# klebgenomics/Kaptive

Measured on AMD Instinct MI355X. Metric: assemblies typed/sec (K+O), higher is better.
Workload: dtype uint16x2 (exact; int32-equivalent); 1 GPU; 10000 synthetic 5 Mbp kpsc assemblies per GPU typed against the synthetic K-locus database, then the O-locus database; one step = all of them, as 10 batches of 1000 through context-owned work buffers; packed assemblies resident in HBM before the timed region; one alignment pass over the genes of both databases, one reduction per database; alignment_passes_per_batch=1, assemblies_per_gpu=10000, assemblies_total=10000, batch=1000, parallelism=1 x independent shard, no collective

## Files before the change

### kaptive_amd/csrc/kp_align.hip

```cpp
#include "kp_host.h"

static const char *const NO_RESULTS = "this batch has no resident alignment results (not aligned yet, or displaced: a context keeps the results of its KP_WORK_SLOTS most recently aligned batches)";

static int enqueue_forked(kp_ctx *ctx, kp_batch *b, KpWork *w, hipStream_t stream) {
    const KpAnchors an = w->anchors();
    const KpTasks tasks = w->tasks();
    const KpJoins joins = w->joins();
    const KpTrace trace = w->trace();
    kp_launch_join_chain(an, tasks, w->groups(), joins, w->d_jscratch.p, ctx->opt.join, w->jstream);
    kp_launch_join_fill(b->view, ctx->genes, joins, trace, ctx->opt.join, w->jstream);
    kp_launch_join_trace(b->view, ctx->genes, joins, tasks, trace, ctx->opt.join, w->jstream);
    kp_launch_task_order(b->view, ctx->genes, an, tasks, stream);
    KP_HIP_CHECK(ctx, hipEventRecord(w->ev[KP_EV_ORDER], stream));
    kp_launch_sw(b->view, ctx->genes, tasks, trace, ctx->max_gene_len > KP_FILL16_MAX_GENE_LEN, ctx->opt.trace_summary, stream, w->ev[KP_EV_FILL]);
    KP_HIP_CHECK(ctx, hipEventRecord(w->ev[KP_EV_TRACEBACK], stream));
    return KP_OK;
}

static int enqueue_align(kp_ctx *ctx, kp_batch *b, KpWork *w) {
    const size_t n_asm = w->n_asm;
    for (auto &e : w->ev)
        if (!e) KP_HIP_CHECK(ctx, hipEventCreate(&e.h));
    if (!w->astream) KP_HIP_CHECK(ctx, hipStreamCreateWithFlags(&w->astream.h, hipStreamNonBlocking));
    if (!w->jstream) {
        KP_HIP_CHECK(ctx, hipStreamCreateWithFlags(&w->jstream.h, hipStreamNonBlocking));
        KP_HIP_CHECK(ctx, hipEventCreateWithFlags(&w->ev_jfork.h, hipEventDisableTiming));
        KP_HIP_CHECK(ctx, hipEventCreateWithFlags(&w->ev_jdone.h, hipEventDisableTiming));
    }
    hipStream_t stream = w->astream;
    const Event *ev = w->ev;
    if ((uint64_t)n_asm * w->anchor_cap > 0xFFFFFFF0ull)
        return kp_fail(ctx, KP_EOVERFLOW, "anchor buffer would exceed 2^32 entries; use smaller batches");
    if (((uint64_t)b->view.total_words << 4) >> KP_CAND_POS_BITS)
        return kp_fail(ctx, KP_EOVERFLOW, "a batch holds at most 2^33 bases (candidate positions); use smaller batches");
    KP_HIP_CHECK(ctx, w->d_anchors_a.reserve(n_asm * w->anchor_cap));
    KP_HIP_CHECK(ctx, w->d_anchors_b.reserve(n_asm * w->anchor_cap));
    KP_HIP_CHECK(ctx, w->d_counts.reserve(w->counts_len()));
// ... 500 lines not shown
```

### kaptive_amd/csrc/kp_ctx.hip

```cpp
#include <cctype>
#include <cstdlib>
#include <mutex>
#include <new>
#include <unordered_map>
#include <sys/mman.h>

#include "kp_host.h"

static std::mutex g_err_mutex;
static std::string g_global_error = "";

std::atomic<long long> g_dev_allocs{0};
bool g_debug_alloc = false;

static std::mutex g_pin_mutex;
struct PinBlock { size_t bytes; bool mapped, locked; };
static std::unordered_map<void *, PinBlock> g_pin_blocks;
static size_t g_pin_bytes = 0;
constexpr size_t HUGE_PAGE = (size_t)2 << 20;
hipError_t pinned_alloc(void **out, size_t bytes) {
    const hipError_t e = hipHostMalloc(out, bytes, hipHostMallocPortable);
    if (e == hipSuccess) {
        std::lock_guard<std::mutex> lk(g_pin_mutex);
        g_pin_blocks[*out] = PinBlock{bytes, false, true};
// ... 72 lines not shown
    const long long x = std::atoll(v);
    return x > 0 ? (uint32_t)x : dflt;
}

static void options_from_env(KpOptions &o) {
    o.anchor_cap = env_u32("KAPTIVE_AMD_ANCHOR_CAP", o.anchor_cap);
    o.tasks_per_asm = env_u32("KAPTIVE_AMD_TASKS_PER_ASM", o.tasks_per_asm);
    o.hit_cap = env_u32("KAPTIVE_AMD_HIT_CAP", o.hit_cap);
    o.trace_kb_per_asm = env_u32("KAPTIVE_AMD_TRACE_KB_PER_ASM", o.trace_kb_per_asm);
    o.trace_set = env_u32("KAPTIVE_AMD_TRACE_KB_PER_ASM", 0) != 0;
    o.cand_cap = env_u32("KAPTIVE_AMD_CAND_CAP", 0);
    o.group_cap = env_u32("KAPTIVE_AMD_GROUP_CAP", o.group_cap);
    o.join_cap = env_u32("KAPTIVE_AMD_JOIN_CAP", o.join_cap);
    o.occ_slots = env_u32("KAPTIVE_AMD_OCC_SLOTS", o.occ_slots);
    o.kept_cap = env_u32("KAPTIVE_AMD_KEPT_CAP", o.kept_cap);
    o.piece_cap = env_u32("KAPTIVE_AMD_PIECE_CAP", o.piece_cap);
    o.prot_cap = env_u32("KAPTIVE_AMD_PROT_CAP", o.prot_cap);
    o.scan_mode = (int)env_u32("KAPTIVE_AMD_SCAN_ABLATE", 0);
    o.library_sort = (int)env_u32("KAPTIVE_AMD_LIBRARY_SORT", 0);
    o.upload_piece_mb = std::max<uint32_t>(1, env_u32("KAPTIVE_AMD_UPLOAD_PIECE_MB", 4096));
    { const char *rb = getenv("KAPTIVE_AMD_READBACK"); o.readback_copy_engine = rb && std::string(rb) == "copy"; }
    o.spin_wait = (int)env_u32("KAPTIVE_AMD_SPIN_WAIT", 0);
    { const char *ts = std::getenv("KAPTIVE_AMD_TRACE_SUMMARY"); o.trace_summary = !(ts && std::string(ts) == "0"); }
    o.join_stats = std::getenv("KAPTIVE_AMD_JOIN_STATS") != nullptr;
    if (const char *e = std::getenv("KAPTIVE_AMD_JOIN_GRID")) std::sscanf(e, "%d,%d,%d,%d", &o.join.fill, &o.join.walk, &o.join.chain, &o.join.chain_large);
    if (const char *e = std::getenv("KAPTIVE_AMD_JOIN_PRIO")) o.join.prio = std::atoi(e);
    if (const char *e = std::getenv("KAPTIVE_AMD_SKIP_JOINS")) o.join.skip = std::atoi(e);
    g_debug_alloc = std::getenv("KAPTIVE_AMD_DEBUG_ALLOC") != nullptr;
}

static void fill_blosum(int8_t *m) {
    static const int8_t b[25][25] = {
        {4, -1, -2, -2, 0, -1, -1, 0, -2, -1, -1, -1, -1, -2, -1, 1, 0, -3, -2, 0, -2, -1, -1, -1, -4},
        {-1, 5, 0, -2, -3, 1, 0, -2, 0, -3, -2, 2, -1, -3, -2, -1, -1, -3, -2, -3, -1, -2, 0, -1, -4},
        {-2, 0, 6, 1, -3, 0, 0, 0, 1, -3, -3, 0, -2, -3, -2, 1, 0, -4, -2, -3, 4, -3, 0, -1, -4},
        {-2, -2, 1, 6, -3, 0, 2, -1, -1, -3, -4, -1, -3, -3, -1, 0, -1, -4, -3, -3, 4, -3, 1, -1, -4},
        {0, -3, -3, -3, 9, -3, -4, -3, -3, -1, -1, -3, -1, -2, -3, -1, -1, -2, -2, -1, -3, -1, -3, -1, -4},
        {-1, 1, 0, 0, -3, 5, 2, -2, 0, -3, -2, 1, 0, -3, -1, 0, -1, -2, -1, -2, 0, -2, 4, -1, -4},
        {-1, 0, 0, 2, -4, 2, 5, -2, 0, -3, -3, 1, -2, -3, -1, 0, -1, -3, -2, -2, 1, -3, 4, -1, -4},
        {0, -2, 0, -1, -3, -2, -2, 6, -2, -4, -4, -2, -3, -3, -2, 0, -2, -2, -3, -3, -1, -4, -2, -1, -4},
        {-2, 0, 1, -1, -3, 0, 0, -2, 8, -3, -3, -1, -2, -1, -2, -1, -2, -2, 2, -3, 0, -3, 0, -1, -4},
        {-1, -3, -3, -3, -1, -3, -3, -4, -3, 4, 2, -3, 1, 0, -3, -2, -1, -3, -1, 3, -3, 3, -3, -1, -4},
        {-1, -2, -3, -4, -1, -2, -3, -4, -3, 2, 4, -2, 2, 0, -3, -2, -1, -2, -1, 1, -4, 3, -3, -1, -4},
        {-1, 2, 0, -1, -3, 1, 1, -2, -1, -3, -2, 5, -1, -3, -1, 0, -1, -3, -2, -2, 0, -3, 1, -1, -4},
        {-1, -1, -2, -3, -1, 0, -2, -3, -2, 1, 2, -1, 5, 0, -2, -1, -1, -1, -1, 1, -3, 2, -1, -1, -4},
        {-2, -3, -3, -3, -2, -3, -3, -3, -1, 0, 0, -3, 0, 6, -4, -2, -2, 1, 3, -1, -3, 0, -3, -1, -4},
// ... 84 lines not shown
    if (ctx) return ctx->error.c_str();
    std::lock_guard<std::mutex> lk(g_err_mutex);
    static thread_local std::string copy;
    copy = g_global_error;
    return copy.c_str();
}

void *kp_ctx_stream(kp_ctx *ctx) { return ctx ? (void *)ctx->stream.h : nullptr; }

int kp_ctx_set_option(kp_ctx *ctx, const char *name, int64_t value) {
    if (!ctx) return kp_fail(nullptr, KP_EINVAL, "null context");
    if (!name || value < 0) return kp_fail(ctx, KP_EINVAL, "bad option");
    const std::string n(name);
    KpOptions &o = ctx->opt;
    if (kp_caps_set_option(o, ctx->learnt, ctx->run_caps, n, value)) return KP_OK;
    if (kp_caps_set_cs_option(ctx->cs_caps, n, value)) return KP_OK;
    if (kp_caps_set_variants_option(ctx->var_caps, n, value)) return KP_OK;
    if (n == "scan_mode") o.scan_mode = (int)value;
    else if (n == "library_sort") o.library_sort = value != 0;
    else if (n == "cigar") o.cigar = value != 0;
    else if (n == "cs") o.cs = value != 0;
    else if (n == "variants") o.variants = value != 0;
    else if (n == "aligned") o.aligned = value != 0;
    else if (n == "upload_piece_mb") o.upload_piece_mb = (uint32_t)std::max<int64_t>(1, std::min<int64_t>(value, 4096));
    else return kp_fail(ctx, KP_EINVAL, "unknown option: " + n);
    return KP_OK;
}

int kp_host_alloc(size_t bytes, void **out) {
    if (!out) return kp_fail(nullptr, KP_EINVAL, "out is null");
    *out = nullptr;
    if (bytes >= 4 * HUGE_PAGE) {
        int rc = kp_host_reserve(bytes, out);
        if (rc == KP_OK && (rc = kp_host_lock(*out)) == KP_OK) return KP_OK;
        if (*out) { pinned_free(*out); *out = nullptr; }
    }
    const hipError_t e = pinned_alloc(out, std::max<size_t>(bytes, 1));
    if (e != hipSuccess) return kp_fail(nullptr, KP_ENOMEM, std::string("hipHostMalloc: ") + hipGetErrorString(e));
    return KP_OK;
}

int kp_host_reserve(size_t bytes, void **out) {
    if (!out) return kp_fail(nullptr, KP_EINVAL, "out is null");
    *out = mapped_alloc(std::max<size_t>(bytes, 1));
    if (!*out) return kp_fail(nullptr, KP_ENOMEM, "mmap failed");
    return KP_OK;
// ... 20 lines not shown
```

### kaptive_amd/csrc/kp_host.h

```cpp
#pragma once

#include <cstring>
#include <memory>
#include "kp_internal.h"
#include "kp_caps.h"
#include "kp_device.h"
#include "kp_reduce_core.h"
static_assert(KP_CAPS_ANCHOR_SUBS == KP_ANCHOR_SUBS, "the policy sizes the scan's sub-slices");

struct KpTypingGroup {
    int32_t gene_lo = 0, gene_hi = 0;
    DevBuf<uint16_t> d_gene_locus, d_gene_pos;
    DevBuf<uint8_t> d_gene_extra, d_prot_db;
    DevBuf<int8_t> d_gene_strand;
    DevBuf<int32_t> d_locus_off, d_locus_len, d_prot_db_off, d_prot_db_len;
    KpTypingDb typing{};
    int max_db_prot_len = 0;
};

struct KpRowLayout {
    bool valid = false;
    size_t n_asm = 0;
    std::vector<int64_t> h_off;
    DevBuf<int64_t> d_off;
// ... 79 lines not shown
    size_t slots() const { return n_asm * (size_t)kept_cap; }
    size_t pairs_len() const { return 4 * slots() + n_asm + 1; }
    KpReduceTables tables() const {
        int32_t *const q = d_pairs.p, *const base = q + 4 * slots();
        return {.best = d_best.p, .keys = d_keys.p, .order = d_order.p, .kept_flag = d_flag.p, .kept = d_kept.p, .kept_cap = kept_cap,
                .pieces = d_pieces.p, .piece_cap = piece_cap, .summary = d_summary.p, .prot = d_prot.p, .prot_cap = prot_cap,
                .q_off = q, .q_len = q + slots(), .t_off = q + 2 * slots(), .t_len = q + 3 * slots(), .pair_base = base, .n_pairs = base + n_asm, .dp8 = d_dp.p};
    }
};

struct kp_batch;

struct KpOptions : KpCapOptions {
    int scan_mode = 0;
    int library_sort = 0;
    uint32_t upload_piece_mb = 4096;
    int readback_copy_engine = 0;
    int spin_wait = 0;
    int cigar = 0;
    int variants = 0;
    int aligned = 0;
    int cs = 0;
    bool trace_summary = true;
    bool join_stats = false;
    KpJoinLaunch join;
};

struct KpInput {
    DevBuf<uint32_t> d_words;
    DevBuf<int64_t> d_asm_word_off;
    DevBuf<int32_t> d_ctg_start, d_ctg_len, d_asm_first_ctg, d_n_runs, d_asm_first_nrun;
    PinnedBlock h_stage;
    Event ready;
};

enum KpPassEvent { KP_EV_START, KP_EV_SCAN, KP_EV_SORT, KP_EV_ORDER, KP_EV_FILL, KP_EV_TRACEBACK, KP_EV_JOINED, KP_EV_END, KP_N_EVENTS };
static_assert(KP_EV_END == 7, "kp_batch_profile returns seven stage times");
enum KpStat { KP_STAT_ANCHORS, KP_STAT_TASKS, KP_STAT_CELLS, KP_STAT_HITS, KP_STAT_RERUNS, KP_N_STATS };
enum KpTopWord { KP_TOP_TRACE = 0, KP_TOP_OCC = 3, KP_TOP_WORDS = 4 };
enum KpJoinCount { KP_JOIN_GROUPS = 0, KP_JOIN_CLASSES = 1, KP_JOIN_COUNTS = 1 + KP_N_CLASSES };
enum KpCandCount { KP_CAND_FRONT, KP_CAND_BACK, KP_CAND_COUNTS };

struct KpWork : KpPassCaps {
    kp_batch *owner = nullptr;
    size_t n_asm = 0;
    KpKeyBits key_bits{16, 30};
// ... 201 lines not shown
```

### kaptive_amd/csrc/kp_internal.h

```cpp
#pragma once

#include <hip/hip_runtime.h>
#include <stdint.h>

#include <string>
#include <vector>

#include "../../include/kaptive_amd.h"

#define KP_FILTER_LOG2 24
__host__ __device__ inline uint32_t kp_filter_block(uint32_t x) { return x & ((1u << (KP_FILTER_LOG2 - 6)) - 1u); }
__host__ __device__ inline uint2 kp_filter_mask2(uint32_t x) {
    uint2 m;
    m.x = 1u << ((x >> 18) & 31u);
    m.y = 1u << ((x >> 23) & 31u);
    return m;
}
__host__ __device__ inline bool kp_filter_test(uint2 got, uint32_t x) {
    return ((got.x >> ((x >> 18) & 31u)) & (got.y >> ((x >> 23) & 31u)) & 1u) != 0u;
}
__host__ __device__ inline uint64_t kp_filter_mask(uint32_t kmer) {
    const uint2 m = kp_filter_mask2(kmer);
    return ((uint64_t)m.y << 32) | m.x;
}
// ... 180 lines not shown
struct KpPieceRows { const kp_piece *pieces; int piece_cap; const int64_t *piece_off; int64_t total; };
struct KpReduceTables {
    const int32_t *best;
    uint64_t *keys;
    uint32_t *order;
    uint8_t *kept_flag;
    kp_kept *kept; int kept_cap;
    kp_piece *pieces; int piece_cap;
    kp_asm_summary *summary;
    uint8_t *prot; int prot_cap;
    int32_t *q_off, *q_len, *t_off, *t_len, *pair_base, *n_pairs;
    int32_t *dp8;
};
struct KpJoinLaunch { int fill = 2048, walk = 512, chain = 2560, chain_large = 512, prio = 1, skip = 0; };

#define KP_ANCHOR_SUBS 64
void kp_launch_scan(const KpBatchView &b, const KpSeedIndex &idx, uint64_t *cand, unsigned long long *n_cand, uint64_t cand_cap,
                    const KpAnchors &an, int ablate_mode, int32_t n_ctg_total, hipStream_t stream, hipEvent_t after_scan);
void kp_launch_anchor_compact(const KpBatchView &b, const KpAnchors &an, hipStream_t stream);
size_t kp_occ_state_words(size_t n_asm, uint32_t occ_slots);
void kp_launch_occ_cut(const KpBatchView &b, const int32_t *gene_len, const KpAnchors &an, uint32_t *occ_keys, uint32_t *occ_cnts,
                       uint32_t *occ_state, unsigned long long *occ_demand, uint32_t occ_slots, uint32_t occ_log2_size, hipStream_t stream);
void kp_launch_chain(const KpBatchView &b, const KpAnchors &an, const KpTasks &tasks, const KpGroups &groups, hipStream_t stream);
void kp_launch_sw(const KpBatchView &b, const KpGenes &genes, const KpTasks &tasks, const KpTrace &trace, bool has_long_genes, bool walk_summaries, hipStream_t stream, hipEvent_t after_fill);
#define KP_ORDER_BUCKETS 65
#define KP_ORDER_COUNTS (2 * KP_N_CLASSES * KP_ORDER_BUCKETS)
#define KP_ORDER_HEAD (KP_ORDER_COUNTS + 2 * KP_N_CLASSES)
void kp_launch_task_order(const KpBatchView &b, const KpGenes &genes, const KpAnchors &an, const KpTasks &tasks, hipStream_t stream);
void kp_launch_join_chain(const KpAnchors &an, const KpTasks &tasks, const KpGroups &groups, const KpJoins &joins, uint8_t *scratch,
                          const KpJoinLaunch &L, hipStream_t stream);
size_t kp_join_chain_scratch_bytes(const KpJoinLaunch &L);
void kp_launch_join_fill(const KpBatchView &b, const KpGenes &genes, const KpJoins &joins, const KpTrace &trace, const KpJoinLaunch &L, hipStream_t stream);
void kp_launch_join_trace(const KpBatchView &b, const KpGenes &genes, const KpJoins &joins, const KpTasks &tasks, const KpTrace &trace,
                          const KpJoinLaunch &L, hipStream_t stream);
void kp_launch_cigar_locate(const KpBatchView &b, const int32_t *gene_len, const KpTasks &tasks, const KpJoins &joins, const KpHitTable &hits,
                            unsigned long long *src, hipStream_t stream);
void kp_launch_cigar_walk(const KpBatchView &b, const KpGenes &genes, const KpTasks &tasks, const KpJoins &joins, const KpTrace &trace, const KpHitTable &hits,
                          const KpHitRows &rows, const unsigned long long *src, const KpPerHit<uint32_t> &cig, bool emit, bool walk_summaries, hipStream_t stream);
void kp_launch_count_scan(const uint32_t *cnt, int64_t n, int64_t *off, hipStream_t stream);
void kp_launch_cs_walk(const KpBatchView &b, const KpGenes &genes, const KpHitTable &hits, const KpHitRows &rows, const KpPerHit<uint32_t> &cig,
                       const KpPerHit<char> &cs, bool emit, hipStream_t stream);
void kp_launch_kept_locate(const KpBatchView &b, const KpHitTable &hits, const KpHitRows &rows, const KpKeptRows &kept, int64_t *src, hipStream_t stream);
void kp_launch_variants_walk(const KpBatchView &b, const KpGenes &genes, const KpPerHit<uint32_t> &cig, const KpKeptRows &kept, const int64_t *src,
                             const KpPerHit<kp_variant> &var, bool emit, hipStream_t stream);
void kp_launch_aligned_count(const KpBatchView &b, const KpGenes &genes, const KpKeptRows &kept, uint32_t *cnt, int64_t *off, hipStream_t stream);
void kp_launch_aligned_emit(const KpBatchView &b, const KpGenes &genes, const KpHitRows &rows, const KpPerHit<uint32_t> &cig, const KpKeptRows &kept,
                            const int64_t *src, const int64_t *off, uint64_t *blocks, kp_aligned_row *out, hipStream_t stream);
// ... 25 lines not shown
```

### kaptive_amd/csrc/kp_sw.hip

```cpp
#include "kp_internal.h"
#include "kp_walk.h"

namespace {

constexpr int CH = 64;
constexpr int OE = KP_GAP_OPEN + KP_GAP_EXT;
constexpr int EX = KP_GAP_EXT;
static_assert(KP_SC_MATCH == 2 && KP_SC_MISMATCH == -4 && KP_SC_N == -1 && OE == 6 && EX == 2,
              "the profile fields and the biases below encode these scores");
static_assert(2 * KP_FILL16_MAX_GENE_LEN + 14 < 0x7C00, "biased scores must stay below the half-precision infinity pattern (pk_max3) "
                                                 "and leave bit 15 of a half-word free for the guard");

constexpr unsigned K1 = 0x00010001u;
constexpr unsigned GUARD = 0x80008000u;
constexpr unsigned CB = 12;
constexpr unsigned ZB = CB - OE;
constexpr unsigned GAP_NONE = (CB - OE - EX) * K1;
constexpr unsigned GAP_EDGE = (CB - OE) * K1;
constexpr unsigned T_OUT = 12u;
constexpr unsigned PROF_OUT = 0u;

template <bool ROW>
__device__ __forceinline__ unsigned from_lower(unsigned v) {
    return (unsigned)(ROW ? __builtin_amdgcn_mov_dpp((int)v, 0x111 , 0xf, 0xf, true)
// ... 152 lines not shown
    s.qb = prof_mine;

    const unsigned eA = bfi_v(first_all, twelve, from_lower<ROW>(pk_max3(s.D.hmoe, s.D.emex, twelve)));
    const unsigned eoA = from_lower<ROW>(sub_v(s.D.hg, s.D.emex));
    dp_cell<FIRST>(s.A, acc[0], s.qb, s.t0, eA, eoA, pk_max(s.B.hmoe, s.B.fmex), sub_v(s.B.hg, s.B.fmex));
    dp_cell<FIRST>(s.B, acc[1], s.qb, s.t1, pk_max3(s.A.hmoe, s.A.emex, twelve), sub_v(s.A.hg, s.A.emex),
                   pk_max(s.C.hmoe, s.C.fmex), sub_v(s.C.hg, s.C.fmex));
    dp_cell<FIRST>(s.C, acc[2], s.qb, s.t2, pk_max3(s.B.hmoe, s.B.emex, twelve), sub_v(s.B.hg, s.B.emex),
                   pk_max(s.D.hmoe, s.D.fmex), sub_v(s.D.hg, s.D.fmex));
    const unsigned fD = bfi_v(last_all, twelve, from_upper<ROW>(pk_max(s.A.hmoe, s.A.fmex)));
    const unsigned foD = from_upper<ROW>(sub_v(s.A.hg, s.A.fmex));
    dp_cell<FIRST>(s.D, acc[3], s.qb, s.t3, pk_max3(s.C.hmoe, s.C.emex, twelve), sub_v(s.C.hg, s.C.emex), fD, foD);

    hs[0] = s.A.hmoe; hs[1] = s.B.hmoe; hs[2] = s.C.hmoe; hs[3] = s.D.hmoe;
    s.t0 = s.t1; s.t1 = s.t2; s.t2 = s.t3;
    s.t3 = t_next;
}

constexpr int PROF_WORDS = 16 * (CH + 4);
constexpr int TCODE_HALVES = 16 * (CH + 3 * 4 + 4 + 4);
constexpr int TWORD_WORDS = 2 * 128;
constexpr int SPREAD_WORDS = 256;

template <int P>
__device__ __forceinline__ void sw_class(const KpBatchView &b, const KpGenes &genes, const KpTask *__restrict__ tasks,
                                         uint32_t n_tasks, const uint32_t *__restrict__ order,
                                         KpSwEnd *__restrict__ ends, uint4 *__restrict__ trace,
                                         unsigned long long *__restrict__ trace_top, uint64_t trace_cap, uint32_t block,
                                         uint32_t n_blocks, unsigned int *__restrict__ next_quad, uint32_t *s_prof_raw,
                                         uint16_t *s_t_raw, uint32_t *s_tw_raw, const uint32_t *s_spread) {
    constexpr int G = 64 / P;
    constexpr int TW = CH + 3 * P + 4;
    constexpr int PAD = (4 - (3 * P + 1) % 4) % 4;
    constexpr int TROW = (TW + PAD + 3) & ~3;
    constexpr int PROW = CH + P;
    static_assert(G * PROW <= PROF_WORDS && G * TROW <= TCODE_HALVES, "LDS carve-up");
    uint32_t(*s_prof)[PROW] = reinterpret_cast<uint32_t(*)[PROW]>(s_prof_raw);
    uint16_t(*s_t)[TROW] = reinterpret_cast<uint16_t(*)[TROW]>(s_t_raw);

    const int lane = threadIdx.x;
    const int g = lane / P, l = lane % P;
    unsigned first_all = l == 0 ? ~0u : 0u, last_all = l == P - 1 ? ~0u : 0u;
    unsigned twelve = CB * K1, fifteen = 15u * K1, one = K1;
    asm volatile("" : "+v"(twelve), "+v"(fifteen), "+v"(one), "+v"(first_all), "+v"(last_all));

    auto take = [&]() -> uint32_t {
        uint32_t q = 0;
        if (lane == 0) q = atomicAdd(next_quad, 1u);
        return (uint32_t)__builtin_amdgcn_readfirstlane((int)q);
    };
    for (uint32_t quad = next_quad ? take() : block; (uint64_t)quad * (2 * G) < n_tasks;
         quad = next_quad ? take() : quad + n_blocks) {
        bool have[2];
// ... 164 lines not shown
                for (int c = 0; c < 4; ++c) np[c] = shl1_or(np[c], pk_min(and_k<KP_PLAIN_MASK>(or_v(held[c], acc[c])), one));
                if (fits && j < tb[0].pieces)
                    trace_x[tb[0].piece_at(j, 0)] = make_uint4(__builtin_amdgcn_perm(acc[0], held[0], 0x05040100u), __builtin_amdgcn_perm(acc[1], held[1], 0x05040100u),
                                                        __builtin_amdgcn_perm(acc[2], held[2], 0x05040100u), __builtin_amdgcn_perm(acc[3], held[3], 0x05040100u));
                if (fits && have[1] && j < tb[1].pieces)
                    trace_y[tb[1].piece_at(j, 0)] = make_uint4(__builtin_amdgcn_perm(acc[0], held[0], 0x07060302u), __builtin_amdgcn_perm(acc[1], held[1], 0x07060302u),
                                                        __builtin_amdgcn_perm(acc[2], held[2], 0x07060302u), __builtin_amdgcn_perm(acc[3], held[3], 0x07060302u));
            }
            {
                const int ch = m0 / CH, up = 8 - ((m_end - m0) >> 3);
                const unsigned sx = (__builtin_amdgcn_perm(np[1], np[0], 0x0c0c0400u) | __builtin_amdgcn_perm(np[3], np[2], 0x04000c0cu)) << up;
                const unsigned sy = (__builtin_amdgcn_perm(np[1], np[0], 0x0c0c0602u) | __builtin_amdgcn_perm(np[3], np[2], 0x06020c0cu)) << up;
                const uint32_t at = (uint32_t)tb[0].sum_at(ch, 0) * 4u;
#ifdef KP_SW_NO_SUMMARY_STORE
                asm volatile("" ::"v"(sx), "v"(sy), "v"(at));
#else
                if (fits && 8 * ch < tb[0].pieces) *reinterpret_cast<uint32_t *>(reinterpret_cast<char *>(trace_x) + (sum_dx + at)) = sx;
                if (fits && have[1] && 8 * ch < tb[1].pieces) *reinterpret_cast<uint32_t *>(reinterpret_cast<char *>(trace_y) + (sum_dy + at)) = sy;
#endif
                np[0] = np[1] = np[2] = np[3] = 0;
            }
        }

#pragma unroll
        for (int h = 0; h < 2; ++h) {
            const unsigned v = (st.best >> (16 * h)) & 0xFFFFu;
            int mstar = (int)((st.brow >> (16 * h)) & 0xFFFFu), cell = 3;
            bool in0 = false;
#pragma unroll
            for (int k = 3; k >= 0; --k)
                if (((st.s0[k] >> (16 * h)) & 0xFFFFu) == v) { cell = k; in0 = true; }
            if (!in0) {
                ++mstar;
#pragma unroll
                for (int k = 2; k >= 0; --k)
                    if (((st.s1[k] >> (16 * h)) & 0xFFFFu) == v) cell = k;
            }
            int eb = 4 * l + cell;
            unsigned key = v > ZB ? ((v - ZB) << 15) | (unsigned)(32767 - (q0[h] + mstar - l)) : 0u;
            if (key == 0u) eb = 4 * l;
            bool sn = saw_n[h];
#pragma unroll
            for (int o = 1; o < P; o <<= 1) {
                const unsigned key2 = (unsigned)__shfl_xor((int)key, o);
                const int eb2 = __shfl_xor(eb, o);
                if (key2 > key || (key2 == key && eb2 < eb)) { key = key2; eb = eb2; }
                sn |= __shfl_xor((int)sn, o) != 0;
            }
            if (have[h] && l == 0) {
                KpSwEnd out;
                out.score = fits ? (int)(key >> 15) : 0;
                out.er = 32767 - (int)(key & 32767u);
                out.eb = eb | (sn ? KP_SWEND_HAS_N : 0);
                out.trace_off = (uint32_t)(h ? toff_y : toff);
                ends[ti[h]] = out;
            }
        }
    }
}

#ifndef KP_SW_WIDE_BLOCKS
#define KP_SW_WIDE_BLOCKS 512
#endif
constexpr uint32_t WIDE_BLOCKS = KP_SW_WIDE_BLOCKS;
#ifndef KP_SW_HELP_BLOCKS
#define KP_SW_HELP_BLOCKS 3072
#endif
constexpr uint32_t HELP_BLOCKS = KP_SW_HELP_BLOCKS;
#ifndef KP_SW_NARROW_BLOCKS_PER_CU
#define KP_SW_NARROW_BLOCKS_PER_CU 32
#endif
constexpr uint32_t NARROW_BLOCKS_PER_CU = KP_SW_NARROW_BLOCKS_PER_CU;

#ifndef KP_SW_WAVES
#define KP_SW_WAVES 3
#endif
#ifndef KP_SW_LDS_PAD
#define KP_SW_LDS_PAD 0
#endif
__global__ __launch_bounds__(64, KP_SW_WAVES) void kp_sw_kernel(KpBatchView b, KpGenes genes, const KpTask *__restrict__ tasks,
                                                   const uint32_t *__restrict__ task_count, uint32_t task_cap,
                                                   const uint32_t *__restrict__ order, KpSwEnd *__restrict__ ends,
                                                   uint4 *__restrict__ trace, unsigned long long *__restrict__ trace_top,
                                                   uint64_t trace_cap) {
    __shared__ __attribute__((aligned(16))) uint32_t s_prof[PROF_WORDS];
    __shared__ __attribute__((aligned(16))) uint16_t s_t[TCODE_HALVES];
    __shared__ uint32_t s_tw[TWORD_WORDS];
    __shared__ uint32_t s_spread[SPREAD_WORDS];
#if KP_SW_LDS_PAD
    __shared__ uint32_t s_pad[KP_SW_LDS_PAD / 4];
    if (task_cap == 0xFFFFFFFFu) { s_pad[threadIdx.x] = blockIdx.x; __syncthreads(); trace_top[3] = s_pad[63 - threadIdx.x]; }
#endif
    for (uint32_t v = threadIdx.x; v < SPREAD_WORDS; v += 64)
        s_spread[v] = 3u * ((v & 3u) | ((v & 0xCu) << 6) | ((v & 0x30u) << 12) | ((v & 0xC0u) << 18));
    const uint32_t blk = blockIdx.x, narrow_end = 3 * WIDE_BLOCKS + 256u * NARROW_BLOCKS_PER_CU;
    const int c = blk < 3 * WIDE_BLOCKS ? 3 - (int)(blk / WIDE_BLOCKS) : blk < narrow_end ? 0 : 3 - (int)((blk - narrow_end) / (HELP_BLOCKS ? HELP_BLOCKS : 1u));
    const size_t off = (size_t)c * task_cap;
    uint32_t n = task_count[c];
    if (n > task_cap) n = task_cap;
    unsigned int *next_quad = reinterpret_cast<unsigned int *>(trace_top + 1) + c;
    if (c == 3) sw_class<32>(b, genes, tasks + off, n, order + off, ends + off, trace, trace_top, trace_cap, 0, 1, next_quad, s_prof, s_t, s_tw, s_spread);
    else if (c == 2) sw_class<16>(b, genes, tasks + off, n, order + off, ends + off, trace, trace_top, trace_cap, 0, 1, next_quad, s_prof, s_t, s_tw, s_spread);
    else if (c == 1) sw_class<8>(b, genes, tasks + off, n, order + off, ends + off, trace, trace_top, trace_cap, 0, 1, next_quad, s_prof, s_t, s_tw, s_spread);
    else sw_class<4>(b, genes, tasks + off, n, order + off, ends + off, trace, trace_top, trace_cap, 0, 1, next_quad, s_prof, s_t, s_tw, s_spread);
}


constexpr int LONG_NEG = -(1 << 29);

template <int P>
__device__ __forceinline__ void sw_long_class(const KpBatchView &b, const KpGenes &genes, const KpTask *__restrict__ tasks,
                                              const uint32_t *__restrict__ order, uint32_t n_tasks, KpSwEnd *__restrict__ ends,
                                              uint4 *__restrict__ trace, unsigned long long *__restrict__ trace_top, uint64_t trace_cap,
                                              uint32_t block, uint32_t n_blocks) {
    constexpr int G = 64 / P;
    const int lane = threadIdx.x, g = lane / P, l = lane % P;
    for (uint32_t quad = block; (uint64_t)quad * G < n_tasks; quad += n_blocks) {
        const uint32_t slot = quad * G + g;
        const bool have = slot < n_tasks;
        const uint32_t ti = have ? order[slot] : 0u;
        KpTask tk;
        tk.asm_id = 0; tk.gs = 0; tk.contig = 0; tk.lo = 0;
        if (have) tk = tasks[ti];
        const KpTaskSeqs s = kp_task_seqs(b, genes, tk.asm_id, tk.gs, tk.contig);
        int q0, r_hi;
        kp_task_rows(tk.lo, 4 * P, s.t.cstart, s.t.cend, have ? s.q.len : 0, &q0, &r_hi);
        const int steps = have ? (r_hi - q0) + P - 1 : 0;
// ... 82 lines not shown
}

__global__ __launch_bounds__(64) void kp_sw_long_kernel(KpBatchView b, KpGenes genes, const KpTask *__restrict__ tasks,
                                                        const uint32_t *__restrict__ order_counts, uint32_t task_cap,
                                                        const uint32_t *__restrict__ order, KpSwEnd *__restrict__ ends,
                                                        uint4 *__restrict__ trace, unsigned long long *__restrict__ trace_top,
                                                        uint64_t trace_cap) {
    const int c = blockIdx.y;
    const uint32_t first = order_counts[c], n = order_counts[KP_N_CLASSES + c];
    if (n == 0) return;
    const size_t off = (size_t)c * task_cap;
    if (c == 3) sw_long_class<32>(b, genes, tasks + off, order + off + first, n, ends + off, trace, trace_top, trace_cap, blockIdx.x, gridDim.x);
    else if (c == 2) sw_long_class<16>(b, genes, tasks + off, order + off + first, n, ends + off, trace, trace_top, trace_cap, blockIdx.x, gridDim.x);
    else if (c == 1) sw_long_class<8>(b, genes, tasks + off, order + off + first, n, ends + off, trace, trace_top, trace_cap, blockIdx.x, gridDim.x);
    else sw_long_class<4>(b, genes, tasks + off, order + off + first, n, ends + off, trace, trace_top, trace_cap, blockIdx.x, gridDim.x);
}

constexpr int TB_THREADS = 256;

__global__ __launch_bounds__(TB_THREADS) void kp_sw_traceback_kernel(KpBatchView b, KpGenes genes, const KpTask *__restrict__ tasks,
                                                              const uint32_t *__restrict__ task_count, uint32_t task_cap,
                                                              const uint32_t *__restrict__ order,
                                                              const KpSwEnd *__restrict__ ends,
                                                              const uint32_t *__restrict__ trace, bool summaries,
                                                              KpSwResult *__restrict__ results) {
    const int cls = blockIdx.y;
    uint32_t n = task_count[cls] + task_count[KP_N_CLASSES + cls];
    if (n > task_cap) n = task_cap;
    const int P = 4 << cls;
    const uint32_t n_iter = (n + 63u) & ~63u;
    for (uint32_t slot = blockIdx.x * blockDim.x + threadIdx.x; slot < n_iter; slot += gridDim.x * blockDim.x) {
        const bool have = slot < n;
        const uint32_t ti = have ? order[(size_t)cls * task_cap + slot] : 0u;
        const size_t at = (size_t)cls * task_cap + ti;
        KpSwEnd e;
        e.score = 0; e.er = 0; e.eb = 0; e.trace_off = 0;
        if (have) e = ends[at];
        KpSwResult out;
        out.score = e.score; out.q_start = out.q_end = out.t_start = out.t_end = out.matches = out.block_len = 0;
        const bool walking = have && e.score >= KP_MIN_DP_SCORE;
        KpTask tk;
        tk.asm_id = 0; tk.gs = 0; tk.contig = 0; tk.lo = 0;
        if (walking) tk = tasks[at];
        const bool has_n = (e.eb & KP_SWEND_HAS_N) != 0;
        const int eb = e.eb & 255;
        const KpTaskSeqs s = kp_task_seqs(b, genes, tk.asm_id, tk.gs, tk.contig);
        int q0 = 0, r_hi = 0;
        if (walking) kp_task_rows(tk.lo, 4 * P, s.t.cstart, s.t.cend, s.q.len, &q0, &r_hi);
        const uint4 *tw = reinterpret_cast<const uint4 *>(trace) + e.trace_off;
        KpBandPath path;
        KpNoVisit nobody;
        kp_band_walk(walking, summaries, tk.lo, P, q0, r_hi, e.er, eb, has_n, tw, s, path, nobody);
        if (!have) continue;
        if (e.score < KP_MIN_DP_SCORE) { results[at] = out; continue; }
        const int matches = has_n ? path.matches : (e.score + 4 * path.diag + path.gap_cost) / 6;
        out.score = e.score + path.credit;
        out.q_start = path.sr; out.q_end = e.er + 1;
        out.t_start = path.sr + tk.lo + path.sb; out.t_end = e.er + tk.lo + eb + 1;
        out.matches = matches; out.block_len = path.cols;
        results[at] = out;
    }
}

}

void kp_launch_sw(const KpBatchView &b, const KpGenes &genes, const KpTasks &t, const KpTrace &trace, bool has_long_genes, bool walk_summaries, hipStream_t stream, hipEvent_t after_fill) {
    const dim3 grid(3 * WIDE_BLOCKS + 256u * NARROW_BLOCKS_PER_CU + 3 * HELP_BLOCKS), block(64);
    hipLaunchKernelGGL(kp_sw_kernel, grid, block, 0, stream, b, genes, t.tasks, t.order_count, t.cap, t.order, t.ends, trace.units, trace.top, trace.cap);
    if (has_long_genes)
        hipLaunchKernelGGL(kp_sw_long_kernel, dim3(256, KP_N_CLASSES), block, 0, stream, b, genes, t.tasks, t.order_count, t.cap, t.order, t.ends,
                           trace.units, trace.top, trace.cap);
    if (after_fill) (void)hipEventRecord(after_fill, stream);
    hipLaunchKernelGGL(kp_sw_traceback_kernel, dim3(2048, KP_N_CLASSES), dim3(TB_THREADS), 0, stream, b, genes, t.tasks, t.order_count,
                       t.cap, t.order, t.ends, reinterpret_cast<const uint32_t *>(trace.units), walk_summaries, t.results);
}
```

### kaptive_amd/csrc/kp_walk.h

```cpp
#pragma once

#include "kp_internal.h"
#include "kp_seqs.h"

#ifndef KP_TRACE_GROUP
#define KP_TRACE_GROUP 2
#endif

enum { KP_COL_M = 0, KP_COL_I = 1, KP_COL_D = 2 };

struct KpNoVisit {
    __device__ __forceinline__ void run(int, int) {}
};

__device__ __forceinline__ KpTaskSeqs kp_task_seqs(const KpBatchView &b, const KpGenes &genes, int asm_id, int gs, int contig) {
    KpTaskSeqs s;
    const int gene = gs >> 1, c_abs = b.asm_first_ctg[asm_id] + contig, r0 = b.asm_first_nrun[asm_id];
    s.q.nib = genes.nib + genes.word_off[(gs & 1) ? genes.n_genes + gene : gene];
    s.q.len = genes.len[gene];
    s.t.words = b.words + b.asm_word_off[asm_id];
    s.t.n_words = (int)(b.asm_word_off[asm_id + 1] - b.asm_word_off[asm_id]);
    s.t.runs = b.n_runs + 2 * (size_t)r0;
    s.t.n_runs = b.asm_first_nrun[asm_id + 1] - r0;
    s.t.cstart = b.ctg_start[c_abs];
    s.t.cend = s.t.cstart + b.ctg_len[c_abs];
    return s;
}

__device__ __forceinline__ unsigned long long kp_trace_take(unsigned long long *trace_top, bool takes, unsigned long long want, int leader) {
    unsigned long long toff = 0;
    if (takes) toff = atomicAdd(trace_top, want);
    return ((unsigned long long)__shfl((unsigned)(toff >> 32), leader) << 32) | __shfl((unsigned)toff, leader);
}
template <int P>
__device__ __forceinline__ void kp_group_best(int &best, int &best_r, int &best_b) {
#pragma unroll
    for (int o = 1; o < P; o <<= 1) {
        const int s2 = __shfl_xor(best, o), r2 = __shfl_xor(best_r, o), b2 = __shfl_xor(best_b, o);
        if (s2 > best || (s2 == best && (r2 < best_r || (r2 == best_r && b2 < best_b)))) { best = s2; best_r = r2; best_b = b2; }
    }
}

__device__ __forceinline__ uint32_t kp_piece_word(const uint4 &v, int k) {
    const uint32_t lo = (k & 1) ? v.y : v.x, hi = (k & 1) ? v.w : v.z;
    return (k & 2) ? hi : lo;
}

constexpr uint32_t KP_PLAIN_MASK = 0xAAAAAAAAu;
constexpr int KP_SUM_PIECES = 8;

struct KpTraceBlock {
    int P;
    int pieces;
    int sum_words;
    __host__ __device__ uint32_t sum_off() const { return (uint32_t)P * (uint32_t)pieces; }
    __host__ __device__ uint32_t units() const { return sum_off() + ((((uint32_t)P * (uint32_t)sum_words + 3u) / 4u + 7u) & ~7u); }
    __host__ __device__ size_t piece_at(int j, int l) const { return (size_t)(j / KP_TRACE_GROUP) * (KP_TRACE_GROUP * P) + KP_TRACE_GROUP * l + j % KP_TRACE_GROUP; }
    __host__ __device__ size_t sum_at(int chunk, int l) const { return (size_t)chunk * P + l; }
};
__host__ __device__ inline KpTraceBlock kp_trace_block(int P, int steps) {
    KpTraceBlock t;
    t.P = P;
    t.pieces = (((steps + 7) >> 3) + 3) & ~3;
    t.sum_words = (t.pieces + KP_SUM_PIECES - 1) / KP_SUM_PIECES;
    return t;
}
__host__ __device__ inline int kp_sum_bit(int cell, int piece) { return 8 * cell + 7 - (piece & 7); }

// ... 55 lines not shown
            if (tag == nxt_tag) {
#pragma unroll
                for (int i = 0; i < TG; ++i) curq[i] = nxtq[i];
            } else {
#pragma unroll
                for (int i = 0; i < TG; ++i) curq[i] = tw[blk.piece_at(grp * TG, l) + i];
            }
            cur_tag = tag;
            int ahead = grp - 1;
            if (summaries && !has_n && grp > 0) {
                bool known;
                const int first = grp * TG;
                int n;
                if (first & 7) n = plain_run(k, first - 1, known);
                else { n = __ffs((int)(((s_low >> (8 * k)) & 255u) | 256u)) - 1; known = n < 8; }
                ahead = known && first - 1 - n >= 0 ? (first - 1 - n) / TG : -1;
            }
            if (ahead >= 0) {
#pragma unroll
                for (int i = 0; i < TG; ++i) nxtq[i] = tw[blk.piece_at(ahead * TG, l) + i];
                nxt_tag = (l << 20) | ahead;
            }
        }
        uint4 cur = (pc & 1) ? curq[1] : curq[0];
        if (TG == 4) {
            const uint4 hi2 = (pc & 1) ? curq[TG - 1] : curq[TG - 2];
            cur = (pc & 2) ? hi2 : cur;
        }
        const uint32_t word = kp_piece_word(cur, k);
        if (!summaries && state == 0 && !has_n && (step & 7) == 7 && (word & KP_PLAIN_MASK) == 0u) {
            cols += 8; diag += 8; r -= 8;
            v.run(KP_COL_M, 8);
            continue;
        }
        const uint32_t half = word >> (16 * ((step >> 2) & 1)), sh = 2 * (step & 3);
        const uint32_t de = ((half >> (8 + sh)) & 3u) ^ 2u, lf = ((half >> sh) & 3u) ^ 2u;
        const uint32_t nib = ((de & 2u) << 2) | ((lf & 2u) << 1) | ((de & 1u) << 1) | (lf & 1u);
        const uint32_t src = (nib & 8u) ? ((nib & 4u) ? 0u : 1u) : ((nib & 4u) ? 2u : 3u);
        if (state == 0) {
            if (src <= 1u) {
                ++cols; ++diag;
                v.run(KP_COL_M, 1);
                if (has_n) {
                    const int qc = s.q.code(r), tc = s.t.at(lo + r + bi);
                    matches += (qc == tc && qc < 4) ? 1 : 0;
                }
                if (src == 1u) { sr = r; sb = bi; walking = false; }
                --r;
            } else {
                state = (int)src - 1;
            }
        } else if (state == 1) {
            ++cols; ++gap; gap_cost += EX;
            v.run(KP_COL_D, 1);
            --bi;
            if (nib & 2u) { state = 0; gap_cost += KP_GAP_OPEN; credit += max(gap - KP_GAP_LONG, 0); gap = 0; }
        } else {
            ++cols; ++gap; gap_cost += EX;
            v.run(KP_COL_I, 1);
            --r; ++bi;
            if (nib & 1u) { state = 0; gap_cost += KP_GAP_OPEN; credit += max(gap - KP_GAP_LONG, 0); gap = 0; }
        }
    }
    out.sr = sr; out.sb = sb; out.cols = cols; out.matches = matches; out.diag = diag; out.gap_cost = gap_cost; out.credit = credit;
}

enum { XT_DIAG = 0, XT_E = 1, XT_F = 2, XT_RESTART = 3, XT_X1 = 4, XT_X2 = 5 };

struct KpJoinPath {
    bool rejected;
    int visited;
    int sr, sb, spk;
    int matches, cols, credit, bonus;
};

template <class V>
__device__ __forceinline__ void kp_join_walk(const KpJoin *J, int k, int P, const KpTaskSeqs &s, const uint4 *trace, KpJoinPath &out, V &v) {
    const int W = 4 * P;
    int pk = k, r = J->end_r[k], bi = J->end_b[k], state = 0, matches = 0, cols = 0, gap = 0, credit = 0;
    int sr = r, sb = bi, spk = k, suf = 0, sufmax = 0, gsum = 0, visited = 1 << k, bonus = 0;
    bool rejected = false;
    int lo = J->lo[pk], q0 = 0, r_hi = 0;
    kp_piece_rows(lo, W, s.t.cstart, s.t.cend, s.q.len, J->r0[pk], J->r1[pk], &q0, &r_hi);
    const uint32_t *tr = reinterpret_cast<const uint32_t *>(trace + J->trace_off[pk]);
    for (;;) {
        const int t = r + lo + bi;
        if (state == 0 && (r < q0 || r >= r_hi || bi < 0 || bi >= W || t < s.t.cstart || t >= s.t.cend)) break;
// ... 50 lines not shown
```

Baseline: 47550 assemblies/s.

## Add opt-in fused traceback walk inside the SW fill kernel

Adds a templated WALK path where the Smith-Waterman fill kernel performs the band traceback walk right after computing end scores, with lanes 0 and 1 each walking one task, so the separate traceback kernel launch can be skipped. The traceback kernel gains a long_only mode to handle only long-gene tasks when fusion is on. Result construction is factored into kp_band_result, and piece-word selection in the walk is rewritten as an unrolled select chain. Fusion defaults off behind an env var or option, so the default path only picks up the select rewrite; when enabled, it risks poor wave utilisation because only two lanes walk.

```diff
diff --git a/kaptive_amd/csrc/kp_align.hip b/kaptive_amd/csrc/kp_align.hip
--- a/kaptive_amd/csrc/kp_align.hip
+++ b/kaptive_amd/csrc/kp_align.hip
@@ -12,7 +12,7 @@
     kp_launch_join_trace(b->view, ctx->genes, joins, tasks, trace, ctx->opt.join, w->jstream);
     kp_launch_task_order(b->view, ctx->genes, an, tasks, stream);
     KP_HIP_CHECK(ctx, hipEventRecord(w->ev[KP_EV_ORDER], stream));
-    kp_launch_sw(b->view, ctx->genes, tasks, trace, ctx->max_gene_len > KP_FILL16_MAX_GENE_LEN, ctx->opt.trace_summary, stream, w->ev[KP_EV_FILL]);
+    kp_launch_sw(b->view, ctx->genes, tasks, trace, ctx->max_gene_len > KP_FILL16_MAX_GENE_LEN, ctx->opt.trace_summary, ctx->opt.fused_traceback, stream, w->ev[KP_EV_FILL]);
     KP_HIP_CHECK(ctx, hipEventRecord(w->ev[KP_EV_TRACEBACK], stream));
     return KP_OK;
 }
diff --git a/kaptive_amd/csrc/kp_ctx.hip b/kaptive_amd/csrc/kp_ctx.hip
--- a/kaptive_amd/csrc/kp_ctx.hip
+++ b/kaptive_amd/csrc/kp_ctx.hip
@@ -118,6 +118,7 @@
     { const char *rb = getenv("KAPTIVE_AMD_READBACK"); o.readback_copy_engine = rb && std::string(rb) == "copy"; }
     o.spin_wait = (int)env_u32("KAPTIVE_AMD_SPIN_WAIT", 0);
     { const char *ts = std::getenv("KAPTIVE_AMD_TRACE_SUMMARY"); o.trace_summary = !(ts && std::string(ts) == "0"); }
+    if (const char *ft = std::getenv("KAPTIVE_AMD_FUSED_TRACEBACK")) o.fused_traceback = std::string(ft) != "0";
     o.join_stats = std::getenv("KAPTIVE_AMD_JOIN_STATS") != nullptr;
     if (const char *e = std::getenv("KAPTIVE_AMD_JOIN_GRID")) std::sscanf(e, "%d,%d,%d,%d", &o.join.fill, &o.join.walk, &o.join.chain, &o.join.chain_large);
     if (const char *e = std::getenv("KAPTIVE_AMD_JOIN_PRIO")) o.join.prio = std::atoi(e);
@@ -248,6 +249,7 @@
     else if (n == "cs") o.cs = value != 0;
     else if (n == "variants") o.variants = value != 0;
     else if (n == "aligned") o.aligned = value != 0;
+    else if (n == "fused_traceback") o.fused_traceback = value != 0;
     else if (n == "upload_piece_mb") o.upload_piece_mb = (uint32_t)std::max<int64_t>(1, std::min<int64_t>(value, 4096));
     else return kp_fail(ctx, KP_EINVAL, "unknown option: " + n);
     return KP_OK;
diff --git a/kaptive_amd/csrc/kp_host.h b/kaptive_amd/csrc/kp_host.h
--- a/kaptive_amd/csrc/kp_host.h
+++ b/kaptive_amd/csrc/kp_host.h
@@ -125,6 +125,7 @@
     int aligned = 0;
     int cs = 0;
     bool trace_summary = true;
+    bool fused_traceback = false;
     bool join_stats = false;
     KpJoinLaunch join;
 };
diff --git a/kaptive_amd/csrc/kp_internal.h b/kaptive_amd/csrc/kp_internal.h
--- a/kaptive_amd/csrc/kp_internal.h
+++ b/kaptive_amd/csrc/kp_internal.h
@@ -226,7 +226,7 @@
 void kp_launch_occ_cut(const KpBatchView &b, const int32_t *gene_len, const KpAnchors &an, uint32_t *occ_keys, uint32_t *occ_cnts,
                        uint32_t *occ_state, unsigned long long *occ_demand, uint32_t occ_slots, uint32_t occ_log2_size, hipStream_t stream);
 void kp_launch_chain(const KpBatchView &b, const KpAnchors &an, const KpTasks &tasks, const KpGroups &groups, hipStream_t stream);
-void kp_launch_sw(const KpBatchView &b, const KpGenes &genes, const KpTasks &tasks, const KpTrace &trace, bool has_long_genes, bool walk_summaries, hipStream_t stream, hipEvent_t after_fill);
+void kp_launch_sw(const KpBatchView &b, const KpGenes &genes, const KpTasks &tasks, const KpTrace &trace, bool has_long_genes, bool walk_summaries, bool fused_traceback, hipStream_t stream, hipEvent_t after_fill);
 #define KP_ORDER_BUCKETS 65
 #define KP_ORDER_COUNTS (2 * KP_N_CLASSES * KP_ORDER_BUCKETS)
 #define KP_ORDER_HEAD (KP_ORDER_COUNTS + 2 * KP_N_CLASSES)
diff --git a/kaptive_amd/csrc/kp_sw.hip b/kaptive_amd/csrc/kp_sw.hip
--- a/kaptive_amd/csrc/kp_sw.hip
+++ b/kaptive_amd/csrc/kp_sw.hip
@@ -198,13 +198,16 @@
 constexpr int TWORD_WORDS = 2 * 128;
 constexpr int SPREAD_WORDS = 256;
 
-template <int P>
+template <bool WALK>
+struct WalkBack {};
+template <int P, bool WALK>
 __device__ __forceinline__ void sw_class(const KpBatchView &b, const KpGenes &genes, const KpTask *__restrict__ tasks,
                                          uint32_t n_tasks, const uint32_t *__restrict__ order,
-                                         KpSwEnd *__restrict__ ends, uint4 *__restrict__ trace,
+                                         KpSwEnd *__restrict__ ends, KpSwResult *__restrict__ results, bool summaries,
+                                         uint4 *__restrict__ trace,
                                          unsigned long long *__restrict__ trace_top, uint64_t trace_cap, uint32_t block,
                                          uint32_t n_blocks, unsigned int *__restrict__ next_quad, uint32_t *s_prof_raw,
-                                         uint16_t *s_t_raw, uint32_t *s_tw_raw, const uint32_t *s_spread) {
+                                         uint16_t *s_t_raw, uint32_t *s_tw_raw, const uint32_t *s_spread, WalkBack<WALK>) {
     constexpr int G = 64 / P;
     constexpr int TW = CH + 3 * P + 4;
     constexpr int PAD = (4 - (3 * P + 1) % 4) % 4;
@@ -415,6 +418,8 @@
             }
         }
 
+        int end_score[2], end_r[2], end_b[2];
+        bool end_n[2];
 #pragma unroll
         for (int h = 0; h < 2; ++h) {
             const unsigned v = (st.best >> (16 * h)) & 0xFFFFu;
@@ -440,14 +445,44 @@
                 if (key2 > key || (key2 == key && eb2 < eb)) { key = key2; eb = eb2; }
                 sn |= __shfl_xor((int)sn, o) != 0;
             }
+            end_score[h] = fits ? (int)(key >> 15) : 0;
+            end_r[h] = 32767 - (int)(key & 32767u);
+            end_b[h] = eb;
+            end_n[h] = sn;
             if (have[h] && l == 0) {
                 KpSwEnd out;
-                out.score = fits ? (int)(key >> 15) : 0;
-                out.er = 32767 - (int)(key & 32767u);
+                out.score = end_score[h];
+                out.er = end_r[h];
                 out.eb = eb | (sn ? KP_SWEND_HAS_N : 0);
                 out.trace_off = (uint32_t)(h ? toff_y : toff);
                 ends[ti[h]] = out;
             }
+        }
+
+        if constexpr (WALK) {
+            __builtin_amdgcn_fence(__ATOMIC_RELEASE, "workgroup");
+            __builtin_amdgcn_fence(__ATOMIC_ACQUIRE, "workgroup");
+            const bool y = l == 1;
+            const bool mine = l < 2 && (y ? have[1] : have[0]);
+            const int w_score = y ? end_score[1] : end_score[0], w_er = y ? end_r[1] : end_r[0], w_eb = y ? end_b[1] : end_b[0];
+            const bool w_n = y ? end_n[1] : end_n[0];
+            const int w_lo = y ? tk[1].lo : tk[0].lo;
+            KpTaskSeqs s;
+            s.q.nib = genes.nib + (y ? q_off[1] : q_off[0]);
+            s.q.len = y ? qlen[1] : qlen[0];
+            s.t.words = b.words + (y ? w_off[1] : w_off[0]);
+            s.t.n_words = (int)(y ? asm_n_words[1] : asm_n_words[0]);
+            s.t.runs = b.n_runs + (y ? run_off[1] : run_off[0]);
+            s.t.n_runs = y ? n_runs[1] : n_runs[0];
+            s.t.cstart = y ? cstart[1] : cstart[0];
+            s.t.cend = y ? cend[1] : cend[0];
+            int w_q0, w_rhi;
+            kp_task_rows(w_lo, 4 * P, s.t.cstart, s.t.cend, s.q.len, &w_q0, &w_rhi);
+            const bool walking = mine && w_score >= KP_MIN_DP_SCORE;
+            KpBandPath path;
+            KpNoVisit nobody;
+            kp_band_walk(walking, summaries, w_lo, P, w_q0, w_rhi, w_er, w_eb, w_n, trace + (y ? toff_y : toff), s, path, nobody);
+            if (mine) results[y ? ti[1] : ti[0]] = kp_band_result(w_score, w_er, w_eb, w_n, w_lo, path);
         }
     }
 }
@@ -471,9 +506,11 @@
 #ifndef KP_SW_LDS_PAD
 #define KP_SW_LDS_PAD 0
 #endif
+template <bool WALK>
 __global__ __launch_bounds__(64, KP_SW_WAVES) void kp_sw_kernel(KpBatchView b, KpGenes genes, const KpTask *__restrict__ tasks,
                                                    const uint32_t *__restrict__ task_count, uint32_t task_cap,
                                                    const uint32_t *__restrict__ order, KpSwEnd *__restrict__ ends,
+                                                   KpSwResult *__restrict__ results, bool summaries,
                                                    uint4 *__restrict__ trace, unsigned long long *__restrict__ trace_top,
                                                    uint64_t trace_cap) {
     __shared__ __attribute__((aligned(16))) uint32_t s_prof[PROF_WORDS];
@@ -492,10 +529,10 @@
     uint32_t n = task_count[c];
     if (n > task_cap) n = task_cap;
     unsigned int *next_quad = reinterpret_cast<unsigned int *>(trace_top + 1) + c;
-    if (c == 3) sw_class<32>(b, genes, tasks + off, n, order + off, ends + off, trace, trace_top, trace_cap, 0, 1, next_quad, s_prof, s_t, s_tw, s_spread);
-    else if (c == 2) sw_class<16>(b, genes, tasks + off, n, order + off, ends + off, trace, trace_top, trace_cap, 0, 1, next_quad, s_prof, s_t, s_tw, s_spread);
-    else if (c == 1) sw_class<8>(b, genes, tasks + off, n, order + off, ends + off, trace, trace_top, trace_cap, 0, 1, next_quad, s_prof, s_t, s_tw, s_spread);
-    else sw_class<4>(b, genes, tasks + off, n, order + off, ends + off, trace, trace_top, trace_cap, 0, 1, next_quad, s_prof, s_t, s_tw, s_spread);
+    if (c == 3) sw_class<32>(b, genes, tasks + off, n, order + off, ends + off, results + off, summaries, trace, trace_top, trace_cap, 0, 1, next_quad, s_prof, s_t, s_tw, s_spread, WalkBack<WALK>{});
+    else if (c == 2) sw_class<16>(b, genes, tasks + off, n, order + off, ends + off, results + off, summaries, trace, trace_top, trace_cap, 0, 1, next_quad, s_prof, s_t, s_tw, s_spread, WalkBack<WALK>{});
+    else if (c == 1) sw_class<8>(b, genes, tasks + off, n, order + off, ends + off, results + off, summaries, trace, trace_top, trace_cap, 0, 1, next_quad, s_prof, s_t, s_tw, s_spread, WalkBack<WALK>{});
+    else sw_class<4>(b, genes, tasks + off, n, order + off, ends + off, results + off, summaries, trace, trace_top, trace_cap, 0, 1, next_quad, s_prof, s_t, s_tw, s_spread, WalkBack<WALK>{});
 }
 
 
@@ -624,22 +661,21 @@
                                                               const uint32_t *__restrict__ task_count, uint32_t task_cap,
                                                               const uint32_t *__restrict__ order,
                                                               const KpSwEnd *__restrict__ ends,
-                                                              const uint32_t *__restrict__ trace, bool summaries,
+                                                              const uint32_t *__restrict__ trace, bool summaries, bool long_only,
                                                               KpSwResult *__restrict__ results) {
     const int cls = blockIdx.y;
     uint32_t n = task_count[cls] + task_count[KP_N_CLASSES + cls];
     if (n > task_cap) n = task_cap;
+    const uint32_t first = long_only ? min(task_count[cls], n) : 0u;
     const int P = 4 << cls;
-    const uint32_t n_iter = (n + 63u) & ~63u;
-    for (uint32_t slot = blockIdx.x * blockDim.x + threadIdx.x; slot < n_iter; slot += gridDim.x * blockDim.x) {
+    const uint32_t n_iter = first + ((n - first + 63u) & ~63u);
+    for (uint32_t slot = first + blockIdx.x * blockDim.x + threadIdx.x; slot < n_iter; slot += gridDim.x * blockDim.x) {
         const bool have = slot < n;
         const uint32_t ti = have ? order[(size_t)cls * task_cap + slot] : 0u;
         const size_t at = (size_t)cls * task_cap + ti;
         KpSwEnd e;
         e.score = 0; e.er = 0; e.eb = 0; e.trace_off = 0;
         if (have) e = ends[at];
-        KpSwResult out;
-        out.score = e.score; out.q_start = out.q_end = out.t_start = out.t_end = out.matches = out.block_len = 0;
         const bool walking = have && e.score >= KP_MIN_DP_SCORE;
         KpTask tk;
         tk.asm_id = 0; tk.gs = 0; tk.contig = 0; tk.lo = 0;
@@ -653,26 +689,21 @@
         KpBandPath path;
         KpNoVisit nobody;
         kp_band_walk(walking, summaries, tk.lo, P, q0, r_hi, e.er, eb, has_n, tw, s, path, nobody);
-        if (!have) continue;
-        if (e.score < KP_MIN_DP_SCORE) { results[at] = out; continue; }
-        const int matches = has_n ? path.matches : (e.score + 4 * path.diag + path.gap_cost) / 6;
-        out.score = e.score + path.credit;
-        out.q_start = path.sr; out.q_end = e.er + 1;
-        out.t_start = path.sr + tk.lo + path.sb; out.t_end = e.er + tk.lo + eb + 1;
-        out.matches = matches; out.block_len = path.cols;
-        results[at] = out;
+        if (have) results[at] = kp_band_result(e.score, e.er, eb, has_n, tk.lo, path);
     }
 }
 
 }
 
-void kp_launch_sw(const KpBatchView &b, const KpGenes &genes, const KpTasks &t, const KpTrace &trace, bool has_long_genes, bool walk_summaries, hipStream_t stream, hipEvent_t after_fill) {
+void kp_launch_sw(const KpBatchView &b, const KpGenes &genes, const KpTasks &t, const KpTrace &trace, bool has_long_genes, bool walk_summaries, bool fused_traceback, hipStream_t stream, hipEvent_t after_fill) {
     const dim3 grid(3 * WIDE_BLOCKS + 256u * NARROW_BLOCKS_PER_CU + 3 * HELP_BLOCKS), block(64);
-    hipLaunchKernelGGL(kp_sw_kernel, grid, block, 0, stream, b, genes, t.tasks, t.order_count, t.cap, t.order, t.ends, trace.units, trace.top, trace.cap);
+    hipLaunchKernelGGL(fused_traceback ? kp_sw_kernel<true> : kp_sw_kernel<false>, grid, block, 0, stream, b, genes, t.tasks, t.order_count, t.cap, t.order, t.ends,
+                       t.results, walk_summaries, trace.units, trace.top, trace.cap);
     if (has_long_genes)
         hipLaunchKernelGGL(kp_sw_long_kernel, dim3(256, KP_N_CLASSES), block, 0, stream, b, genes, t.tasks, t.order_count, t.cap, t.order, t.ends,
                            trace.units, trace.top, trace.cap);
     if (after_fill) (void)hipEventRecord(after_fill, stream);
-    hipLaunchKernelGGL(kp_sw_traceback_kernel, dim3(2048, KP_N_CLASSES), dim3(TB_THREADS), 0, stream, b, genes, t.tasks, t.order_count,
-                       t.cap, t.order, t.ends, reinterpret_cast<const uint32_t *>(trace.units), walk_summaries, t.results);
-}
+    if (!fused_traceback || has_long_genes)
+        hipLaunchKernelGGL(kp_sw_traceback_kernel, dim3(fused_traceback ? 64 : 2048, KP_N_CLASSES), dim3(TB_THREADS), 0, stream, b, genes, t.tasks, t.order_count,
+                           t.cap, t.order, t.ends, reinterpret_cast<const uint32_t *>(trace.units), walk_summaries, fused_traceback, t.results);
+}
diff --git a/kaptive_amd/csrc/kp_walk.h b/kaptive_amd/csrc/kp_walk.h
--- a/kaptive_amd/csrc/kp_walk.h
+++ b/kaptive_amd/csrc/kp_walk.h
@@ -42,8 +42,9 @@
 }
 
 __device__ __forceinline__ uint32_t kp_piece_word(const uint4 &v, int k) {
-    const uint32_t lo = (k & 1) ? v.y : v.x, hi = (k & 1) ? v.w : v.z;
-    return (k & 2) ? hi : lo;
+    const uint32_t x = v.x, y = v.y, z = v.z, w = v.w;
+    const uint32_t lo = (k & 1) ? +y : +x, hi = (k & 1) ? +w : +z;
+    return (k & 2) ? +hi : +lo;
 }
 
 constexpr uint32_t KP_PLAIN_MASK = 0xAAAAAAAAu;
@@ -145,12 +146,12 @@
                 nxt_tag = (l << 20) | ahead;
             }
         }
-        uint4 cur = (pc & 1) ? curq[1] : curq[0];
-        if (TG == 4) {
-            const uint4 hi2 = (pc & 1) ? curq[TG - 1] : curq[TG - 2];
-            cur = (pc & 2) ? hi2 : cur;
-        }
-        const uint32_t word = kp_piece_word(cur, k);
+        uint32_t word = kp_piece_word(curq[0], k);
+#pragma unroll
+        for (int i = 1; i < TG; ++i) {
+            const uint32_t wi = kp_piece_word(curq[i], k);
+            word = pc % TG == i ? wi : word;
+        }
         if (!summaries && state == 0 && !has_n && (step & 7) == 7 && (word & KP_PLAIN_MASK) == 0u) {
             cols += 8; diag += 8; r -= 8;
             v.run(KP_COL_M, 8);
@@ -186,6 +187,18 @@
         }
     }
     out.sr = sr; out.sb = sb; out.cols = cols; out.matches = matches; out.diag = diag; out.gap_cost = gap_cost; out.credit = credit;
+}
+
+__device__ __forceinline__ KpSwResult kp_band_result(int score, int er, int eb, bool has_n, int lo, const KpBandPath &path) {
+    KpSwResult out;
+    out.score = score; out.q_start = out.q_end = out.t_start = out.t_end = out.matches = out.block_len = 0;
+    if (score < KP_MIN_DP_SCORE) return out;
+    out.score = score + path.credit;
+    out.q_start = path.sr; out.q_end = er + 1;
+    out.t_start = path.sr + lo + path.sb; out.t_end = er + lo + eb + 1;
+    out.matches = has_n ? path.matches : (score + 4 * path.diag + path.gap_cost) / 6;
+    out.block_len = path.cols;
+    return out;
 }
 
 enum { XT_DIAG = 0, XT_E = 1, XT_F = 2, XT_RESTART = 3, XT_X1 = 4, XT_X2 = 5 };
```

Measured after the change: 46820 assemblies/s. -1.5%, worse.
